# SebastianHafner/multimodal_siamese_cd

Measured on AMD Instinct MI355X. Metric: image-pairs/sec training step, 256×256 SAR+optical Siamese U-Net, 1/2/4/8 MI355X, higher is better.
Workload: dtype f32 (h2 split-fp16); 1 GPU; baseline_siamese: siameseunet TOPOLOGY [64, 128, 256, 512], 5-ch SAR+optical, 256x256, bs=32/GPU, conv math h2, fp32 activation storage, train step incl. AdamW; global_batch=32, tile=256, parallelism=dp1

## Files before the change

### include/scd.h

```cpp
#ifndef SCD_H_
#define SCD_H_

#include <stddef.h>
#include <stdint.h>

#ifdef __cplusplus
extern "C" {
#endif

typedef void *scd_stream_t;

enum scd_status {
    SCD_OK = 0,
    SCD_ERR_ARG = -1,
    SCD_ERR_ALIGN = -2,
    SCD_ERR_LAUNCH = -3,
    SCD_ERR_DEVICE = -4,
    SCD_ERR_WORKSPACE = -5,
};

enum scd_dtype {
    SCD_DT_F32 = 0,
    SCD_DT_BF16 = 1
};

typedef struct scd_nhwc {
    void *data;
    int32_t n, h, w, c, ldc;
    int32_t dtype;
} scd_nhwc_t;

const char *scd_version(void);
const char *scd_last_error(void);
int scd_device_check(int device);

int scd_pack_nchw(const float *src, int32_t n, int32_t c, int32_t h, int32_t w, int32_t c_begin,
                  int32_t c_count, scd_nhwc_t dst, float *bound, scd_stream_t stream);

typedef struct scd_pack_job {
    const float *w;
    float *out;
    uint16_t *split;
    int32_t co, ci, ci_pad, mode;
    int32_t math;
} scd_pack_job_t;
int scd_pack_conv3x3_multi(const scd_pack_job_t *jobs, int32_t n, scd_stream_t stream);
int scd_pack_conv3x3(const float *w, int32_t co, int32_t ci, int32_t ci_pad, int32_t mode, float *out,
                     scd_stream_t stream);

int scd_pack_convT2x2(const float *w, int32_t ci, int32_t co, int32_t mode, float *out, scd_stream_t stream);
int scd_pack_convT2x2_multi(const scd_pack_job_t *jobs, int32_t n, scd_stream_t stream);

enum scd_conv_math {
    SCD_MATH_F32 = 0,
    SCD_MATH_X3 = 1,
    SCD_MATH_BF16 = 2,
    SCD_MATH_X5 = 3,
    SCD_MATH_H2 = 4
};
#define SCD_ABI_VERSION 11
int scd_abi_version(void);
#define SCD_TUNE_HALO16_CFG(id)   ((uint32_t)((id) + 1))
#define SCD_TUNE_HALO16_OFF       0xFu
#define SCD_TUNE_HALO16_MASK      0xFu
#define SCD_TUNE_HALO16_WRING     0x8u
#define SCD_TUNE_H2_TILE_2X2      (1u << 4)
#define SCD_TUNE_H2_TILE64_2X2    (1u << 5)
#define SCD_TUNE_H2_NO_PRESCALE   (1u << 6)
#define SCD_TUNE_NO_XCD_REMAP     (1u << 7)
#define SCD_TUNE_HALO_ORDER_M     (1u << 8)
#define SCD_TUNE_W16_LAYOUT_2X2   (1u << 9)
#define SCD_TUNE_WGRAD_R64        (1u << 10)
#define SCD_TUNE_BF16_1XN         (1u << 11)
#define SCD_TUNE_X3_TILE(t)       ((uint32_t)(t) << 12)
#define SCD_TUNE_X3_TILE_MASK     (0xFu << 12)
#define SCD_TUNE_C16_TILES(k)     ((uint32_t)(k) << 16)
#define SCD_TUNE_C16_TILES_MASK   (0xFu << 16)
#define SCD_TUNE_HALO16_DB_OFF    (1u << 20)
#define SCD_TUNE_HALO16_DB_ON     (1u << 21)
#define SCD_TUNE_NO_GATHER16      (1u << 22)
#define SCD_TUNE_NO_WGRAD_C16     (1u << 23)
#define SCD_TUNE_NO_WGRAD_H2      (1u << 24)
#define SCD_TUNE_NO_HALO16_C16    (1u << 25)
#define SCD_TUNE_NO_HALO          (1u << 26)
#define SCD_TUNE_H2_TILE64_128    (1u << 28)
#define SCD_TUNE_WGRAD16_REGSTAGE (1u << 30)
int scd_split_bf16x3(const float *src, int64_t n, uint16_t *dst, scd_stream_t stream);
size_t scd_split_frag_bytes(int32_t n_out, int32_t K);
int scd_split_bf16x3_frag(const float *w, int32_t n_out, int32_t K, uint16_t *dst, scd_stream_t stream);
int scd_split_h2_frag(const float *w, int32_t n_out, int32_t K, uint16_t *dst, scd_stream_t stream);

typedef struct scd_bn_bwd_tiles {
    scd_nhwc_t y;
    int32_t nseg;
    const float *save_mean, *save_invstd, *scale, *shift;
    float *rec;
} scd_bn_bwd_tiles_t;

typedef struct scd_igemm {
    scd_nhwc_t src;
    int32_t out_h, out_w;
    int32_t stride;
    int32_t ntaps;
    int8_t dy[9], dx[9];
    const float *wpk;
    int32_t n_out;
    const float *bias;
    scd_nhwc_t dst;
    int32_t store_mode;
    const uint16_t *wsplit;
    float *stat_rec;
    const float *in_scale;
    const float *in_shift;
    int32_t in_nseg;
    const scd_bn_bwd_tiles_t *bn_bwd;
    const float *src_bound;
    float *dst_bound;
    int32_t math;
    uint32_t tune;
    const float *dst_bound_seed;
} scd_igemm_t;

int scd_conv_igemm(const scd_igemm_t *d, scd_stream_t stream);
int scd_igemm_arith(const scd_igemm_t *d);
int scd_igemm_bn_bwd_tiles(const scd_igemm_t *d, int32_t *tile_pixels);
int scd_igemm_input_bn_supported(const scd_igemm_t *d);
int scd_igemm_stat_tiles(const scd_igemm_t *d, int32_t *tile_pixels);

enum scd_igemm_family {
    SCD_KERNEL_F32 = 0,
    SCD_KERNEL_X3 = 1,
    SCD_KERNEL_HALO32 = 2,
    SCD_KERNEL_HALO16 = 3,
    SCD_KERNEL_HALO16_C16 = 4,
    SCD_KERNEL_GATHER16 = 5
};
typedef struct scd_igemm_kernel {
    int32_t family;
    int32_t layout;
    int32_t block_pixels;
    int32_t block_channels;
    int32_t tile_width;
    int32_t np;
    int32_t db;
    int32_t sb;
    int32_t in_bn;
    int32_t wl;
} scd_igemm_kernel_t;
int scd_igemm_kernel(const scd_igemm_t *d, scd_igemm_kernel_t *out);

typedef struct scd_wgrad {
    scd_nhwc_t rows;
    scd_nhwc_t src;
    int32_t stride;
    int32_t ntaps;
    int8_t dy[9], dx[9];
    const float *src_scale;
    const float *src_shift;
    int32_t src_nseg;
    const float *rows_bound;
    const float *src_bound;
    scd_nhwc_t rows_y;
    int32_t rows_nseg;
    const float *rows_mean, *rows_invstd, *rows_gamma, *rows_scale, *rows_shift, *rows_coef;
    int32_t math;
    uint32_t tune;
    float *src_colsum;
// ... 253 lines not shown
```

### multimodal_siamese_cd_amd/csrc/conv_halo16.hip

```cpp
#include "x3_common.h"

namespace scd {

template <int CTRL>
__device__ __forceinline__ float dpp_mov(float x) {
    return __builtin_bit_cast(float, __builtin_amdgcn_update_dpp(0, __builtin_bit_cast(int, x), CTRL, 0xf, 0xf, false));
}
__device__ __forceinline__ float row16_sum(float x) {
    x += dpp_mov<0x140>(x);
    x += dpp_mov<0x141>(x);
    x += dpp_mov<0xB1>(x);
    x += dpp_mov<0x4E>(x);
    return x;
}

__device__ __forceinline__ f32x4 row16_sum4(f32x4 v) {
    float a, b, c, d;
    asm volatile(
        "s_nop 1\n\t"
        "v_add_f32_dpp %0, %4, %4 row_mirror row_mask:0xf bank_mask:0xf bound_ctrl:1\n\t"
        "v_add_f32_dpp %1, %5, %5 row_mirror row_mask:0xf bank_mask:0xf bound_ctrl:1\n\t"
        "v_add_f32_dpp %2, %6, %6 row_mirror row_mask:0xf bank_mask:0xf bound_ctrl:1\n\t"
        "v_add_f32_dpp %3, %7, %7 row_mirror row_mask:0xf bank_mask:0xf bound_ctrl:1\n\t"
        "v_add_f32_dpp %0, %0, %0 row_half_mirror row_mask:0xf bank_mask:0xf bound_ctrl:1\n\t"
// ... 1040 lines not shown
}

template <int TW>
static void launch_c16_tw(const IgemmArgs &b, dim3 grid, hipStream_t s) {
    switch (c16_planes(b)) {
        case 1:
            if (b.sb)
                hipLaunchKernelGGL((igemm_halo16_c16<TW, 1, true>), grid, dim3(256), 0, s, b);
            else
                hipLaunchKernelGGL((igemm_halo16_c16<TW, 1>), grid, dim3(256), 0, s, b);
            break;
        case 4: hipLaunchKernelGGL((igemm_halo16_c16<TW, 4>), grid, dim3(256), 0, s, b); break;
        case 5: hipLaunchKernelGGL((igemm_halo16_c16<TW, 5>), grid, dim3(256), 0, s, b); break;
        default: hipLaunchKernelGGL((igemm_halo16_c16<TW, 3>), grid, dim3(256), 0, s, b);
    }
}

template <int TW>
static int c16_resident(const IgemmArgs &b) {
    static int cache[4] = {0, 0, 0, 0};
    const int pl = c16_planes(b);
    const int k = pl == 1 ? 0 : pl == 5 ? 1 : pl == 4 ? 3 : 2;
    if (cache[k] > 0) return cache[k];
    const void *fn = k == 0   ? reinterpret_cast<const void *>(&igemm_halo16_c16<TW, 1>)
                     : k == 1 ? reinterpret_cast<const void *>(&igemm_halo16_c16<TW, 5>)
                     : k == 3 ? reinterpret_cast<const void *>(&igemm_halo16_c16<TW, 4>)
                              : reinterpret_cast<const void *>(&igemm_halo16_c16<TW, 3>);
    int per_cu = 0, cus = 0, dev = 0;
    if (hipGetDevice(&dev) != hipSuccess ||
        hipDeviceGetAttribute(&cus, hipDeviceAttributeMultiprocessorCount, dev) != hipSuccess ||
        hipOccupancyMaxActiveBlocksPerMultiprocessor(&per_cu, fn, 256, 0) != hipSuccess || per_cu < 1 || cus < 1) {
        (void)hipGetLastError();
        cache[k] = 2 * 256;
        return cache[k];
    }
    cache[k] = per_cu * cus;
    return cache[k];
}

void launch_halo16_c16(const IgemmArgs &a, int tw, hipStream_t s) {
    IgemmArgs b = a;
    b.grid_m = a.n_img * (a.ho / (128 / tw)) * (a.wo / tw);
    b.grid_n = (a.n_out + 63) / 64;
    b.remap = 0;
    const int64_t ntile = int64_t(b.grid_m) * b.grid_n;
    const int cap = tw == 64 ? c16_resident<64>(a) : tw == 32 ? c16_resident<32>(a) : c16_resident<16>(a);
    const int kt = int((a.tune & SCD_TUNE_C16_TILES_MASK) >> 16);
    const int k = kt == 0 ? 4 : kt == 15 ? 0 : kt;
    const int64_t blocks = k >= 1 ? (ntile + k - 1) / k : (ntile < cap ? ntile : cap);
    const dim3 grid(static_cast<unsigned>(blocks));
    if (tw == 64)
        launch_c16_tw<64>(b, grid, s);
    else if (tw == 32)
        launch_c16_tw<32>(b, grid, s);
    else
        launch_c16_tw<16>(b, grid, s);
}

namespace {
constexpr int kW16RS = 160;

#ifndef SCD_WGRAD_ROW_WALK
#define SCD_WGRAD_ROW_WALK 0
#endif
__device__ __forceinline__ int patch_y0(int pr, int pw_n, int ph_n, int ph) {
    return SCD_WGRAD_ROW_WALK ? (pr / pw_n) * ph : (pr - (pr / ph_n) * ph_n) * ph;
}
__device__ __forceinline__ int patch_x0(int pr, int pw_n, int ph_n, int pw) {
    return SCD_WGRAD_ROW_WALK ? (pr - (pr / pw_n) * pw_n) * pw : (pr / ph_n) * pw;
}

template <int NP>
constexpr int w16_xp() { return NP == 1 ? 1 : (NP == 5 || NP == 2 || NP == 4) ? 2 : 3; }
template <int NP>
constexpr int w16_dp() { return NP == 1 ? 1 : (NP == 2 || NP == 4) ? 2 : 3; }

template <int LC>
struct W16L {
    static constexpr int CB = LC ? 1 : 2;
    static constexpr int RB = LC ? 4 : 2;
    static constexpr int NH = 9 * CB;
};

template <int T, int CB, int PB, int HW_, int NP>
__device__ __forceinline__ void w16_read_x(s16x4 (&f)[6], uint32_t xbase) {
    constexpr int toff = (T / 3) * HW_ + (T % 3);
    tr_read<0 * PB + toff * kW16RS + CB * 32>(f[0], xbase);
    tr_read<0 * PB + (toff + 8) * kW16RS + CB * 32>(f[1], xbase);
    if constexpr (w16_xp<NP>() >= 2) {
        tr_read<1 * PB + toff * kW16RS + CB * 32>(f[2], xbase);
        tr_read<1 * PB + (toff + 8) * kW16RS + CB * 32>(f[3], xbase);
    }
    if constexpr (w16_xp<NP>() == 3) {
        tr_read<2 * PB + toff * kW16RS + CB * 32>(f[4], xbase);
        tr_read<2 * PB + (toff + 8) * kW16RS + CB * 32>(f[5], xbase);
    }
}

template <int I, int PA, int NRB, int DP, int RSD>
__device__ __forceinline__ void w16_read_dy(bf16x8 (&dv)[3][NRB], uint32_t dbase) {
    if constexpr (I < DP * NRB) {
        constexpr int p = I / NRB, rb = I % NRB;
        s16x4 lo, hi;
        tr_read<p * PA + rb * 32>(lo, dbase);
        tr_read<p * PA + 8 * RSD + rb * 32>(hi, dbase);
        dv[p][rb] = cat8(lo, hi);
        w16_read_dy<I + 1, PA, NRB, DP, RSD>(dv, dbase);
    }
}

template <int T, int CB, int WAIT, int NP, int LC>
__device__ __forceinline__ void w16_half(f32x4 (&acc)[9][W16L<LC>::CB][W16L<LC>::RB],
                                         bf16x8 (&dv)[3][W16L<LC>::RB], s16x4 (&f)[6]) {
    bf16x8 x0 = cat8(f[0], f[1]), x1 = cat8(f[2], f[3]), x2 = cat8(f[4], f[5]);
    if constexpr (NP == 2 || NP == 4) {
        lds_wait<WAIT>(x0, x1);
        if (T == 0 && CB == 0) {
#pragma unroll
            for (int rb = 0; rb < W16L<LC>::RB; ++rb) lds_wait<WAIT>(dv[0][rb], dv[1][rb]);
        }
        const u32x4 xh = __builtin_bit_cast(u32x4, x0), xm = __builtin_bit_cast(u32x4, x1);
        const u32x4 xh_lo = NP == 4 ? f16_down11(xh) : xh;
#pragma unroll
        for (int rb = 0; rb < W16L<LC>::RB; ++rb) {
            const u32x4 dh = __builtin_bit_cast(u32x4, dv[0][rb]), dm = __builtin_bit_cast(u32x4, dv[1][rb]);
            acc[T][CB][rb] = mfma16_f16(xm, dh, acc[T][CB][rb]);
            acc[T][CB][rb] = mfma16_f16(xh_lo, dm, acc[T][CB][rb]);
            acc[T][CB][rb] = mfma16_f16(xh, dh, acc[T][CB][rb]);
        }
        return;
    }
    if constexpr (NP != 1) {
        if constexpr (NP == 3)
            lds_wait<WAIT>(x0, x1, x2);
        else
            lds_wait<WAIT>(x0, x1);
        if (T == 0 && CB == 0) {
#pragma unroll
            for (int rb = 0; rb < W16L<LC>::RB; ++rb) lds_wait<WAIT>(dv[0][rb], dv[1][rb], dv[2][rb]);
        }
    } else {
        lds_wait<WAIT>(x0);
        if (T == 0 && CB == 0) {
#pragma unroll
            for (int rb = 0; rb < W16L<LC>::RB; ++rb) lds_wait<WAIT>(dv[0][rb]);
        }
    }
#pragma unroll
    for (int rb = 0; rb < W16L<LC>::RB; ++rb) {
        if constexpr (NP != 1) {
            acc[T][CB][rb] = __builtin_amdgcn_mfma_f32_16x16x32_bf16(x1, dv[1][rb], acc[T][CB][rb], 0, 0, 0);
            acc[T][CB][rb] = __builtin_amdgcn_mfma_f32_16x16x32_bf16(x0, dv[2][rb], acc[T][CB][rb], 0, 0, 0);
            if constexpr (NP == 3)
                acc[T][CB][rb] = __builtin_amdgcn_mfma_f32_16x16x32_bf16(x2, dv[0][rb], acc[T][CB][rb], 0, 0, 0);
            acc[T][CB][rb] = __builtin_amdgcn_mfma_f32_16x16x32_bf16(x0, dv[1][rb], acc[T][CB][rb], 0, 0, 0);
            acc[T][CB][rb] = __builtin_amdgcn_mfma_f32_16x16x32_bf16(x1, dv[0][rb], acc[T][CB][rb], 0, 0, 0);
        }
        acc[T][CB][rb] = __builtin_amdgcn_mfma_f32_16x16x32_bf16(x0, dv[0][rb], acc[T][CB][rb], 0, 0, 0);
    }
}

template <int H, int PB, int HW_, int NP, int LC>
__device__ __forceinline__ void w16_chain(f32x4 (&acc)[9][W16L<LC>::CB][W16L<LC>::RB], bf16x8 (&dv)[3][W16L<LC>::RB],
                                          s16x4 (&f0)[6], s16x4 (&f1)[6], uint32_t xbase) {
    constexpr int NCB = W16L<LC>::CB, NH = W16L<LC>::NH;
    if constexpr (H < NH) {
        s16x4 (&f)[6] = (H & 1) ? f1 : f0;
        w16_half<H / NCB, H % NCB, (H == NH - 1 ? 0 : 2 * w16_xp<NP>()), NP, LC>(acc, dv, f);
        if constexpr (H + 2 < NH) w16_read_x<(H + 2) / NCB, (H + 2) % NCB, PB, HW_, NP>(f, xbase);
        w16_chain<H + 1, PB, HW_, NP, LC>(acc, dv, f0, f1, xbase);
    }
}

constexpr int kW16PH = 2, kW16PW = 16;

struct W16Block {
    int split, ct, r0, c0;
    int pw_n, ph_n, pimg, pbeg, pend;
    bool writer;
};
template <int ROWS, int COLS, bool RBN>
__device__ __forceinline__ W16Block w16_block(const WgradArgs &a) {
    W16Block b;
    const uint32_t per_split = COLS == 16 ? uint32_t(a.grid_r) : uint32_t(a.grid_r * a.grid_j);
    const uint32_t L = a.remap ? xcd_swizzle(blockIdx.x, gridDim.x) : blockIdx.x;
    b.split = int(L / per_split);
    const int rem = int(L - uint32_t(b.split) * per_split);
    b.ct = COLS == 16 ? 0 : rem / a.grid_r;
    b.r0 = (rem - b.ct * a.grid_r) * ROWS;
    b.c0 = b.ct * COLS;
    b.pw_n = a.wo / kW16PW;
    b.ph_n = a.ho / kW16PH;
    b.pimg = b.pw_n * b.ph_n;
    const int npatch = a.n_img_w * b.pimg;
    b.pbeg = b.split * a.kchunk;
    b.pend = min(npatch, b.pbeg + a.kchunk);
    b.writer = RBN && a.rows_out && b.ct == 0;
    return b;
}

template <int NCB, int NRB>
__device__ __forceinline__ void w16_store_slabs(f32x4 (&acc)[9][NCB][NRB], const WgradArgs &a, int split, int r0w, int w16,
                                                int c0w, int g) {
    float *slab = a.slabs + size_t(split) * a.R * a.Ng;
#pragma unroll
    for (int t = 0; t < 9; ++t)
#pragma unroll
        for (int cb = 0; cb < NCB; ++cb)
#pragma unroll
            for (int r = 0; r < NRB; ++r) {
                const int row = r0w + 16 * r + w16;
                const int col = c0w + 16 * cb + 4 * g;
                gstore4(slab + size_t(row) * a.Ng + t * a.C + col, acc[t][cb][r]);
            }
}
}

template <int NP, int LC, int RG, bool SB = false, bool RBN = false>
__global__ __launch_bounds__(256 * RG, 2 / RG) void wgrad_halo16_x3(WgradArgs a) {
    static_assert(!SB || NP == 1, "bf16 storage runs the bf16 arithmetic");
    static_assert(!RBN || (LC == 1 && (NP == 1 || NP == 4)), "rows transform: h2 / bf16, along-c layout");
    constexpr uint32_t EB = SB ? 2u : 4u;
    constexpr int NT = 256 * RG;
    constexpr int PH = kW16PH, PW = kW16PW, P = PH * PW;
    constexpr int HW_ = PW + 2, HP = (PH + 2) * HW_;
    constexpr int RS = kW16RS;
    constexpr int RSD = 128 * RG + 32;
    constexpr int CQ = 16 * RG;
    constexpr int PA = P * RSD, PB = HP * RS;
    constexpr int A_CH = P * CQ, B_CH = HP * 16;
    constexpr int A_PER = A_CH / NT, B_PER = (B_CH + NT - 1) / NT;
    static_assert(RG == 1 || (RG == 2 && LC == 1), "128-row blocks use the along-c wave layout");
    static_assert(NP == 1 || NP == 2 || NP == 3 || NP == 4 || NP == 5, "x3, x5, bf16 or h2");
    constexpr bool H2 = NP == 2 || NP == 4;
    constexpr int DP = w16_dp<NP>();
    constexpr int XP = w16_xp<NP>();
    constexpr int STAGE = DP * PA + XP * PB;
    constexpr int RBLK = 64 * RG;
    constexpr int COEF = RBN ? 2 * 7 * RBLK * 4 : 0;
    constexpr bool YDMA = RBN && H2;
    constexpr int YST = YDMA ? A_PER * NT * 16 : 0;
    __shared__ __attribute__((aligned(16))) unsigned char smem[STAGE + COEF + YST];
    float ds = 1.f, ds_inv = 1.f, xs = 1.f, xs_inv = 1.f;
    if constexpr (H2) {
        h2_scale(*a.rows_bound, ds, ds_inv);
        h2_scale(*a.src_bound, xs, xs_inv);
    }

    const int tid = threadIdx.x, lane = tid & 63, wid = tid >> 6;
    constexpr int NCB = W16L<LC>::CB, NRB = W16L<LC>::RB;
    const int wi = LC ? (RG == 1 ? 0 : wid >> 2) : wid >> 1, wj = LC ? (RG == 1 ? wid : wid & 3) : wid & 1;
    const W16Block blk = w16_block<RBLK, 64, RBN>(a);
    const int r0 = blk.r0, c0 = blk.c0, pimg = blk.pimg, pbeg = blk.pbeg, pend = blk.pend;

    const __amdgpu_buffer_rsrc_t rs_rows = make_rsrc(a.rows, a.rows_bytes);
    const __amdgpu_buffer_rsrc_t rs_src = make_rsrc(a.src, a.src_bytes);
    const __amdgpu_buffer_rsrc_t rs_y = make_rsrc(RBN ? a.rows_y : a.rows, RBN ? a.y_bytes : 0u);
    const bool writer = blk.writer;
    float omax = 0.f;

    StageT<SB> ra[A_PER], rb[B_PER], ya[RBN && !YDMA ? A_PER : 1];
    unsigned char *const ystage = smem + STAGE + COEF;
    const int wave_u = __builtin_amdgcn_readfirstlane(wid);
    f32x4 x_sc, x_sh;
    uint32_t x_valid = 0;
    int st_img = 0, st_y0 = 0, st_x0 = 0;
    auto load_patch = [&](int pi) {
        const int img = pi / pimg, pr = pi - img * pimg;
        if (a.src_scale) {
            const int ch = (img / a.src_seg_imgs) * a.C + c0 + (tid & 15) * 4;
            x_sc = gload4(a.src_scale + ch);
            x_sh = gload4(a.src_shift + ch);
        }
        x_valid = 0;
        const int y0 = patch_y0(pr, blk.pw_n, blk.ph_n, PH), x0 = patch_x0(pr, blk.pw_n, blk.ph_n, PW);
        st_img = img;
        st_y0 = y0;
        st_x0 = x0;
#pragma unroll
        for (int i = 0; i < A_PER; ++i) {
            const int e = tid + i * NT, q = e / CQ, cq = e % CQ;
            const int py = q >> 4, px = q & 15;
            const int pix = (img * a.ho + y0 + py) * a.wo + x0 + px;
            if constexpr (YDMA)
                __builtin_amdgcn_global_load_lds(
                    (const __attribute__((address_space(1))) void *)(a.rows_y + size_t(pix) * a.ldc_y + r0 + cq * 4),
                    (__attribute__((address_space(3))) void *)(ystage + (i * NT + wave_u * 64) * 16), 16, 0, 0);
            ra[i] = bload_q<SB>(rs_rows, uint32_t(pix * a.ldc_r + r0 + cq * 4) * EB);
            if constexpr (RBN && !YDMA) ya[i] = bload_q<SB>(rs_y, uint32_t(pix * a.ldc_y + r0 + cq * 4) * EB);
        }
#pragma unroll
        for (int i = 0; i < B_PER; ++i) {
            const int e = tid + i * NT, hp = e >> 4, cq = e & 15;
            const int hy = hp / HW_, hx = hp - (hp / HW_) * HW_;
            const int sy = y0 - 1 + hy, sx = x0 - 1 + hx;
            const bool v = e < B_CH && unsigned(sy) < unsigned(a.hs) && unsigned(sx) < unsigned(a.ws);
            x_valid |= uint32_t(v) << i;
            rb[i] = bload_q<SB>(rs_src, v ? uint32_t(((img * a.hs + sy) * a.ws + sx) * a.ldc_s + c0 + cq * 4) * EB : kOOB);
        }
    };
    auto store_patch = [&]() {
        const f32x4 sc = H2 ? x_sc * xs : x_sc, sh = H2 ? x_sh * xs : x_sh;
        if constexpr (YDMA) asm volatile("s_waitcnt vmcnt(0)" ::: "memory");
#pragma unroll
        for (int i = 0; i < A_PER; ++i) {
            const int e = tid + i * NT;
            const int o = (e / CQ) * RSD + (e % CQ) * 8;
            u32x2 h, m, l;
            if constexpr (RBN) {
                const int cq = e % CQ, q = e / CQ;
                const float *cf =
                    reinterpret_cast<const float *>(smem + STAGE) + (st_img / a.rows_seg_imgs) * 7 * RBLK + cq * 4;
                const f32x4 mu = *reinterpret_cast<const f32x4 *>(cf), iv = *reinterpret_cast<const f32x4 *>(cf + RBLK);
                const f32x4 sc = *reinterpret_cast<const f32x4 *>(cf + 2 * RBLK);
                const f32x4 sf = *reinterpret_cast<const f32x4 *>(cf + 3 * RBLK);
                const f32x4 k1 = *reinterpret_cast<const f32x4 *>(cf + 4 * RBLK);
                const f32x4 k2 = *reinterpret_cast<const f32x4 *>(cf + 5 * RBLK);
                const f32x4 mul = *reinterpret_cast<const f32x4 *>(cf + 6 * RBLK);
                f32x4 yv;
                if constexpr (YDMA)
                    yv = *reinterpret_cast<const f32x4 *>(ystage + e * 16);
                else
                    yv = stage_f32<SB>(ya[i]);
                f32x4 dv = bn_bwd_dy4(yv, stage_f32<SB>(ra[i]), mu, iv, sc, sf, k1, k2, mul);
                if constexpr (SB) {
                    const u32x2 bits = pk_bf16x4(dv);
                    ra[i] = bits;
                    dv = unpk_bf16x4(bits);
                } else {
                    ra[i] = dv;
                }
                if (writer) {
                    const int pix = (st_img * a.ho + st_y0 + (q >> 4)) * a.wo + st_x0 + (q & 15);
                    const size_t idx = size_t(pix) * a.ldc_o + r0 + cq * 4;
                    if constexpr (SB)
                        *reinterpret_cast<u32x2 *>(static_cast<unsigned short *>(a.rows_out) + idx) = ra[i];
                    else
                        gstore4(static_cast<float *>(a.rows_out) + idx, dv);
                    omax = fmaxf(omax, fmaxf(fmaxf(fabsf(dv[0]), fabsf(dv[1])), fmaxf(fabsf(dv[2]), fabsf(dv[3]))));
                }
            }
            if constexpr (H2) {
                if constexpr (NP == 4)
                    split2h_pre(ra[i] * ds, h, m);
                else
                    split2h(ra[i] * ds, h, m);
                *reinterpret_cast<u32x2 *>(smem + PA + o) = m;
            } else if constexpr (DP == 3) {
                split3(ra[i], h, m, l);
                *reinterpret_cast<u32x2 *>(smem + PA + o) = m;
                *reinterpret_cast<u32x2 *>(smem + 2 * PA + o) = l;
            } else {
                h = stage_bits<SB>(ra[i]);
            }
            *reinterpret_cast<u32x2 *>(smem + o) = h;
        }
#pragma unroll
        for (int i = 0; i < B_PER; ++i)
            if constexpr (SB) {
                if (tid + i * NT < B_CH) {
                    u32x2 h = rb[i];
                    if (a.src_scale) {
                        const bool v = (x_valid >> i) & 1u;
                        f32x4 x = unpk_bf16x4(rb[i]);
#pragma unroll
                        for (int q = 0; q < 4; ++q) x[q] = v ? fmaxf(fmaf(x[q], sc[q], sh[q]), 0.f) : 0.f;
                        h = pk_bf16x4(x);
                    }
                    const int e = tid + i * NT;
                    *reinterpret_cast<u32x2 *>(smem + DP * PA + (e >> 4) * RS + (e & 15) * 8) = h;
                }
            } else if (tid + i * NT < B_CH) {
                u32x2 h, m, l;
                if (a.src_scale) {
                    const bool v = (x_valid >> i) & 1u;
#pragma unroll
                    for (int q = 0; q < 4; ++q) rb[i][q] = v ? fmaxf(fmaf(rb[i][q], sc[q], sh[q]), 0.f) : 0.f;
                } else if constexpr (H2) {
                    rb[i] *= xs;
                }
                const int e = tid + i * NT;
                const int o = DP * PA + (e >> 4) * RS + (e & 15) * 8;
                if constexpr (H2) {
                    split2h(rb[i], h, m);
                    *reinterpret_cast<u32x2 *>(smem + PB + o) = m;
                } else if constexpr (XP >= 2) {
                    split3(rb[i], h, m, l);
                    *reinterpret_cast<u32x2 *>(smem + PB + o) = m;
                    if constexpr (XP == 3) *reinterpret_cast<u32x2 *>(smem + 2 * PB + o) = l;
                } else {
                    h[0] = cvt_pk_bf16(rb[i][0], rb[i][1]);
                    h[1] = cvt_pk_bf16(rb[i][2], rb[i][3]);
                }
                *reinterpret_cast<u32x2 *>(smem + o) = h;
            }
    };

    f32x4 acc[9][NCB][NRB];
#pragma unroll
    for (int t = 0; t < 9; ++t)
#pragma unroll
        for (int i = 0; i < NCB; ++i)
#pragma unroll
            for (int j = 0; j < NRB; ++j) acc[t][i][j] = f32x4{0.f, 0.f, 0.f, 0.f};

    const int g = lane >> 4, w16 = lane & 15;
    const int py = g >> 1, pxq = 4 * (g & 1) + (w16 >> 2);
    const uint32_t dbase = lds_addr(smem) + (py * PW + pxq) * RSD + (16 * NRB * wi + 4 * (w16 & 3)) * 2;
    const uint32_t xbase = lds_addr(smem) + DP * PA + (py * HW_ + pxq) * RS + (16 * NCB * wj + 4 * (w16 & 3)) * 2;

    if constexpr (RBN) {
        float *cf = reinterpret_cast<float *>(smem + STAGE);
        const int nsl = a.n_img_w / a.rows_seg_imgs;
        for (int e = tid; e < nsl * RBLK; e += NT) {
            const int sg = e / RBLK, r = e - sg * RBLK, o = sg * a.R + r0 + r;
            const float iv = a.rbn_inv[o];
            float *c = cf + sg * 7 * RBLK + r;
            c[0] = a.rbn_mean[o];
            c[RBLK] = iv;
            c[2 * RBLK] = a.rbn_scale[o];
            c[3 * RBLK] = a.rbn_shift[o];
            c[4 * RBLK] = a.rbn_coef[2 * o];
            c[5 * RBLK] = a.rbn_coef[2 * o + 1];
            c[6 * RBLK] = (a.rbn_gamma ? a.rbn_gamma[r0 + r] : 1.f) * iv;
        }
        __syncthreads();
    }
    if (pbeg < pend) {
        load_patch(pbeg);
        store_patch();
        __syncthreads();
        for (int pi = pbeg; pi < pend; ++pi) {
            const bool more = pi + 1 < pend;
            if (more) load_patch(pi + 1);
            bf16x8 dv[3][NRB];
            w16_read_dy<0, PA, NRB, DP, RSD>(dv, dbase);
            s16x4 f0[6], f1[6];
            w16_read_x<0 / NCB, 0 % NCB, PB, HW_, NP>(f0, xbase);
            w16_read_x<1 / NCB, 1 % NCB, PB, HW_, NP>(f1, xbase);
            w16_chain<0, PB, HW_, NP, LC>(acc, dv, f0, f1, xbase);
            if (more) {
                __syncthreads();
                store_patch();
                __syncthreads();
            }
        }
    }

    if constexpr (H2) {
        const float k = ds_inv * xs_inv;
#pragma unroll
        for (int t = 0; t < 9; ++t)
#pragma unroll
            for (int cb = 0; cb < NCB; ++cb)
#pragma unroll
                for (int r = 0; r < NRB; ++r) acc[t][cb][r] *= k;
    }
    if (writer && a.rows_out_bound) wave_max_bound(a.rows_out_bound, omax);
    w16_store_slabs(acc, a, blk.split, r0 + 16 * NRB * wi, w16, c0 + 16 * NCB * wj, g);
}

namespace {
constexpr int kDmaSink = 1024;
}
#ifndef SCD_WGRAD16_DMA_NB
#define SCD_WGRAD16_DMA_NB 4
#endif
#ifndef SCD_WGRAD16_DMA_TRANSFORMS
#define SCD_WGRAD16_DMA_TRANSFORMS 1
#endif
#ifndef SCD_WGRAD16_DMA_NB_XT
#define SCD_WGRAD16_DMA_NB_XT 5
#endif

template <int RG, int NB, bool XT = false, bool RBN = false>
__global__ __launch_bounds__(256 * RG, 2 / RG) void wgrad_halo16_dma(WgradArgs a) {
    constexpr int NT = 256 * RG, NW = NT / 64;
    constexpr int PH = kW16PH, PW = kW16PW, P = PH * PW;
    constexpr int HW_ = PW + 2, HP = (PH + 2) * HW_;
    constexpr int RS = kW16RS;
    constexpr int RSD = 128 * RG + 32;
    constexpr int PA = P * RSD, PB = HP * RS;
    constexpr int PA_K = (PA + 1023) / 1024, PB_K = (PB + 1023) / 1024;
    constexpr int NPC = PA_K + PB_K + (RBN ? PA_K : 0);
    constexpr int PPW = (NPC + NW - 1) / NW;
    constexpr int STAGE = NPC * 1024;
    constexpr int DCH = 8 * RG;
    constexpr int RBLK = 64 * RG;
    constexpr int NCB = W16L<1>::CB, NRB = W16L<1>::RB;
    constexpr bool TR = XT || RBN;
    static_assert(NB >= (TR ? 3 : 2) && NB <= 6, "ring depth");
    static_assert(!RBN || (P * DCH) % NT == 0, "rows transform: whole 16-byte chunks per thread");
    constexpr int RCH = RBN ? P * DCH / NT : 0;
    constexpr int CFX = XT ? 2 * 2 * 64 * 4 : 0;
    constexpr int CFR = RBN ? 2 * 7 * RBLK * 4 : 0;
    static_assert(NB * STAGE + kDmaSink + CFX + CFR <= 160 * 1024,
                  "ring depth NB: NB patch buffers and the coefficient tables exceed the CU's 160 KB of LDS");
    __shared__ __attribute__((aligned(16))) unsigned char smem[NB * STAGE + kDmaSink + CFX + CFR];

    const int tid = threadIdx.x, lane = tid & 63, wid = tid >> 6;
    const int wave_u = __builtin_amdgcn_readfirstlane(wid);
    const int wi = RG == 1 ? 0 : wid >> 2, wj = RG == 1 ? wid : wid & 3;
    const W16Block blk = w16_block<RBLK, 64, RBN>(a);
    const int r0 = blk.r0, c0 = blk.c0, pimg = blk.pimg, pbeg = blk.pbeg, pend = blk.pend;
    const bool writer = blk.writer;
    float omax = 0.f;

    const __amdgpu_buffer_rsrc_t rs_rows = make_rsrc(a.rows, a.rows_bytes);
    const __amdgpu_buffer_rsrc_t rs_src = make_rsrc(a.src, a.src_bytes);
    const __amdgpu_buffer_rsrc_t rs_y = make_rsrc(RBN ? a.rows_y : a.rows, RBN ? a.y_bytes : 0u);
    int rel[PPW], x_hy[PPW], x_hx[PPW], kind[PPW];
#pragma unroll
    for (int k = 0; k < PPW; ++k) {
        const int u = k * NW + wave_u;
        kind[k] = 2;
        rel[k] = x_hy[k] = x_hx[k] = 0;
        const bool is_y = RBN && u >= PA_K + PB_K && u < NPC;
        if (u < PA_K || is_y) {
            const int b = (is_y ? u - PA_K - PB_K : u) * 1024 + lane * 16;
            const int row = b / RSD, ch = (b - row * RSD) / 16;
            if (row < P && ch < DCH) {
                kind[k] = 0;
                rel[k] = ((row >> 4) * a.wo + (row & 15)) * (is_y ? a.ldc_y : a.ldc_r) + r0 + 8 * ch;
            }
        } else if (u < PA_K + PB_K) {
            const int b = (u - PA_K) * 1024 + lane * 16;
// ... 148 lines not shown
            cfx[sg * 128 + c] = a.src_scale[sg * a.C + c0 + c];
            cfx[sg * 128 + 64 + c] = a.src_shift[sg * a.C + c0 + c];
        }
    }
    if constexpr (RBN) {
        const int nsl = a.n_img_w / a.rows_seg_imgs;
        for (int e = tid; e < nsl * RBLK; e += NT) {
            const int sg = e / RBLK, r = e - sg * RBLK, o = sg * a.R + r0 + r;
            const float iv = a.rbn_inv[o];
            float *c = cfr + sg * 7 * RBLK + r;
            c[0] = a.rbn_mean[o];
            c[RBLK] = iv;
            c[2 * RBLK] = a.rbn_scale[o];
            c[3 * RBLK] = a.rbn_shift[o];
            c[4 * RBLK] = a.rbn_coef[2 * o];
            c[5 * RBLK] = a.rbn_coef[2 * o + 1];
            c[6 * RBLK] = (a.rbn_gamma ? a.rbn_gamma[r0 + r] : 1.f) * iv;
        }
    }

    const int wst = writer ? RCH : 0;
    Cursor ci = cursor_at(pbeg), ct1 = ci;
#pragma unroll
    for (int k = 0; k < NB - 1; ++k)
        if (pbeg + k < pend) {
            issue(ci, k);
            advance(ci);
        }
    if constexpr (TR) {
        if (pbeg < pend) {
            const int ahead = min(NB - 2, pend - 1 - pbeg);
            if (ahead >= 3)
                asm volatile("s_waitcnt vmcnt(%0)" ::"n"(3 * PPW) : "memory");
            else if (ahead == 2)
                asm volatile("s_waitcnt vmcnt(%0)" ::"n"(2 * PPW) : "memory");
            else if (ahead == 1)
                asm volatile("s_waitcnt vmcnt(%0)" ::"n"(PPW) : "memory");
            else
                asm volatile("s_waitcnt vmcnt(0)" ::: "memory");
            lds_barrier();
            transform(ct1, 0);
            advance(ct1);
        }
    }
    int slot = 0;
    for (int pi = pbeg; pi < pend; ++pi) {
        const int ahead = TR ? (pi + 1 < pend ? min(NB - 3, pend - 2 - pi) : -1) : min(NB - 2, pend - 1 - pi);
        if (wst == 0) {
            if (ahead >= 4)
                asm volatile("s_waitcnt vmcnt(%0)" ::"n"(4 * PPW) : "memory");
            else if (ahead == 3)
                asm volatile("s_waitcnt vmcnt(%0)" ::"n"(3 * PPW) : "memory");
            else if (ahead == 2)
                asm volatile("s_waitcnt vmcnt(%0)" ::"n"(2 * PPW) : "memory");
            else if (ahead == 1)
                asm volatile("s_waitcnt vmcnt(%0)" ::"n"(PPW) : "memory");
            else if (ahead == 0)
                asm volatile("s_waitcnt vmcnt(0)" ::: "memory");
        } else if constexpr (RBN) {
            if (ahead >= 3)
                asm volatile("s_waitcnt vmcnt(%0)" ::"n"(3 * PPW + RCH) : "memory");
            else if (ahead == 2)
                asm volatile("s_waitcnt vmcnt(%0)" ::"n"(2 * PPW + RCH) : "memory");
            else if (ahead == 1)
                asm volatile("s_waitcnt vmcnt(%0)" ::"n"(PPW + RCH) : "memory");
            else if (ahead == 0)
                asm volatile("s_waitcnt vmcnt(%0)" ::"n"(RCH) : "memory");
        }
        lds_barrier();
        if (pi + NB - 1 < pend) {
            issue(ci, slot == 0 ? NB - 1 : slot - 1);
            advance(ci);
        }
        if constexpr (TR) {
            if (pi + 1 < pend) {
                transform(ct1, slot == NB - 1 ? 0 : slot + 1);
                advance(ct1);
            }
        }
        const uint32_t bo = uint32_t(slot * STAGE);
        bf16x8 dv[3][NRB];
        w16_read_dy<0, PA_K * 1024, NRB, 1, RSD>(dv, dbase + bo);
        s16x4 f0[6], f1[6];
        w16_read_x<0, 0, PB_K * 1024, HW_, 1>(f0, xbase + bo);
        w16_read_x<1, 0, PB_K * 1024, HW_, 1>(f1, xbase + bo);
        w16_chain<0, PB_K * 1024, HW_, 1, 1>(acc, dv, f0, f1, xbase + bo);
        slot = slot == NB - 1 ? 0 : slot + 1;
    }
    asm volatile("s_waitcnt vmcnt(0)" ::: "memory");
    if (writer && a.rows_out_bound) wave_max_bound(a.rows_out_bound, omax);
    w16_store_slabs(acc, a, blk.split, r0 + 16 * NRB * wi, w16, c0 + 16 * NCB * wj, g);
}

namespace {
constexpr int kC16RS = 32;

template <int T, int PB, int HW_, int NP>
__device__ __forceinline__ void c16_read_x(s16x4 (&f)[6], uint32_t xbase) {
    constexpr int toff = (T / 3) * HW_ + (T % 3);
    tr_read<0 * PB + toff * kC16RS>(f[0], xbase);
    tr_read<0 * PB + (toff + 8) * kC16RS>(f[1], xbase);
    if constexpr (w16_xp<NP>() >= 2) {
        tr_read<1 * PB + toff * kC16RS>(f[2], xbase);
        tr_read<1 * PB + (toff + 8) * kC16RS>(f[3], xbase);
    }
    if constexpr (w16_xp<NP>() == 3) {
        tr_read<2 * PB + toff * kC16RS>(f[4], xbase);
        tr_read<2 * PB + (toff + 8) * kC16RS>(f[5], xbase);
    }
}

template <int T, int WAIT, int NP>
__device__ __forceinline__ void c16_tap(f32x4 (&acc)[9], bf16x8 (&dv)[3], s16x4 (&f)[6]) {
    bf16x8 x0 = cat8(f[0], f[1]), x1 = cat8(f[2], f[3]), x2 = cat8(f[4], f[5]);
    if constexpr (NP == 4) {
        lds_wait<WAIT>(x0, x1);
        if (T == 0) lds_wait<WAIT>(dv[0], dv[1]);
        const u32x4 xh = __builtin_bit_cast(u32x4, x0), xm = __builtin_bit_cast(u32x4, x1);
        const u32x4 dh = __builtin_bit_cast(u32x4, dv[0]), dm = __builtin_bit_cast(u32x4, dv[1]);
        acc[T] = mfma16_f16(xm, dh, acc[T]);
        acc[T] = mfma16_f16(f16_down11(xh), dm, acc[T]);
        acc[T] = mfma16_f16(xh, dh, acc[T]);
        return;
    }
    if constexpr (NP != 1) {
        if constexpr (NP == 3)
            lds_wait<WAIT>(x0, x1, x2);
        else
            lds_wait<WAIT>(x0, x1);
        if (T == 0) lds_wait<WAIT>(dv[0], dv[1], dv[2]);
    } else {
        lds_wait<WAIT>(x0, dv[0]);
    }
    if constexpr (NP != 1) {
        acc[T] = __builtin_amdgcn_mfma_f32_16x16x32_bf16(x1, dv[1], acc[T], 0, 0, 0);
        acc[T] = __builtin_amdgcn_mfma_f32_16x16x32_bf16(x0, dv[2], acc[T], 0, 0, 0);
        if constexpr (NP == 3) acc[T] = __builtin_amdgcn_mfma_f32_16x16x32_bf16(x2, dv[0], acc[T], 0, 0, 0);
        acc[T] = __builtin_amdgcn_mfma_f32_16x16x32_bf16(x0, dv[1], acc[T], 0, 0, 0);
        acc[T] = __builtin_amdgcn_mfma_f32_16x16x32_bf16(x1, dv[0], acc[T], 0, 0, 0);
    }
    acc[T] = __builtin_amdgcn_mfma_f32_16x16x32_bf16(x0, dv[0], acc[T], 0, 0, 0);
}

template <int T, int PB, int HW_, int NP>
__device__ __forceinline__ void c16_chain(f32x4 (&acc)[9], bf16x8 (&dv)[3], s16x4 (&f0)[6], s16x4 (&f1)[6],
                                          uint32_t xbase) {
    if constexpr (T < 9) {
        s16x4 (&f)[6] = (T & 1) ? f1 : f0;
        c16_tap<T, (T == 8 ? 0 : 2 * w16_xp<NP>()), NP>(acc, dv, f);
        if constexpr (T + 2 < 9) c16_read_x<T + 2, PB, HW_, NP>(f, xbase);
        c16_chain<T + 1, PB, HW_, NP>(acc, dv, f0, f1, xbase);
    }
}
}

template <int NP, bool RBN, bool SB = false>
__global__ __launch_bounds__(256, 2) void wgrad_halo16_c16(WgradArgs a) {
    static_assert(!SB || NP == 1, "bf16 storage runs the bf16 arithmetic");
    constexpr uint32_t EB = SB ? 2u : 4u;
    constexpr int PH = kW16PH, PW = kW16PW, P = PH * PW;
    constexpr int HW_ = PW + 2, HP = (PH + 2) * HW_;
    constexpr int RS = kW16RS, RSX = kC16RS;
    constexpr int PA = P * RS, PB = HP * RSX;
    constexpr int A_CH = P * 16, B_CH = HP * 4;
    constexpr int A_PER = A_CH / 256, B_PER = (B_CH + 255) / 256;
    static_assert(NP == 1 || NP == 3 || NP == 4 || NP == 5, "x3, x5, bf16 or h2");
    constexpr bool H2 = NP == 4;
    constexpr int DP = w16_dp<NP>();
    constexpr int XP = w16_xp<NP>();
// ... 339 lines not shown
```

### multimodal_siamese_cd_amd/hip.py

```python
from __future__ import annotations

import collections
import contextlib
import contextvars
import ctypes
import os
from ctypes import POINTER, c_char_p, c_float, c_int, c_int8, c_int32, c_int64, c_size_t, c_uint8, c_uint32, c_void_p

import torch

LIB_PATH = os.environ.get("SCD_LIB") or os.path.join(os.path.dirname(os.path.abspath(__file__)), "_lib", "libscd.so")


class NHWC(ctypes.Structure):

    _fields_ = [("data", c_void_p), ("n", c_int32), ("h", c_int32), ("w", c_int32), ("c", c_int32), ("ldc", c_int32),
                ("dtype", c_int32)]


DT_F32, DT_BF16 = 0, 1
_VIEW_DTYPES = {torch.float32: (DT_F32, 4), torch.bfloat16: (DT_BF16, 2)}


class BNBWD(ctypes.Structure):
# ... 365 lines not shown
    out = torch.empty(ci * co * 4, device=w.device, dtype=torch.float32)
    _check(lib().scd_pack_convT2x2(w.contiguous().data_ptr(), ci, co, mode, out.data_ptr(), _stream()),
           "scd_pack_convT2x2")
    return _attach_split(out, 4 * co, ci, 1) if mode == 0 else _attach_split(out, ci, 4 * co, 4)


def pack_convT2x2_multi(jobs) -> list:
    if not jobs:
        return []
    split = conv_math() != 'f32'
    m = _MATH_NAMES[conv_math()]
    outs, keep, arr = [], [], (PACKJOB * len(jobs))()
    for i, (w, mode) in enumerate(jobs):
        ci, co = w.shape[0], w.shape[1]
        w = w.contiguous()
        n_out, K = (4 * co, ci) if mode == 0 else (ci, 4 * co)
        out = torch.empty(ci * co * 4, device=w.device, dtype=torch.float32)
        sp = None
        if split and K % 16 == 0:
            sp = torch.empty(lib().scd_split_frag_bytes(n_out, K) // 2, dtype=torch.int16, device=w.device)
            out._x3 = sp
        keep.append(w)
        arr[i] = PACKJOB(w.data_ptr(), out.data_ptr(), _ptr(sp), co, ci, ci, mode, m)
        outs.append(out)
    _check(lib().scd_pack_convT2x2_multi(ctypes.cast(arr, c_void_p), len(jobs), _stream()), "scd_pack_convT2x2_multi")
    return outs


def split_bf16x3(src: torch.Tensor) -> torch.Tensor:
    n = src.numel()
    dst = torch.empty(3 * n, dtype=torch.int16, device=src.device)
    _check(lib().scd_split_bf16x3(src.data_ptr(), n, dst.data_ptr(), _stream()), "scd_split_bf16x3")
    return dst


def split_h2_frag(wpk: torch.Tensor, n_out: int, K: int) -> torch.Tensor:
    nbytes = lib().scd_split_frag_bytes(n_out, K)
    dst = torch.empty(nbytes // 2, dtype=torch.int16, device=wpk.device)
    _check(lib().scd_split_h2_frag(wpk.data_ptr(), n_out, K, dst.data_ptr(), _stream()), "scd_split_h2_frag")
    return dst


def split_bf16x3_frag(wpk: torch.Tensor, n_out: int, K: int) -> torch.Tensor:
    nbytes = lib().scd_split_frag_bytes(n_out, K)
    dst = torch.empty(nbytes // 2, dtype=torch.int16, device=wpk.device)
    _check(lib().scd_split_bf16x3_frag(wpk.data_ptr(), n_out, K, dst.data_ptr(), _stream()), "scd_split_bf16x3_frag")
    return dst


def h2_weight_format(K: int, ntaps: int) -> bool:
    if conv_math() != 'h2' or ntaps not in (9, 1, 4) or K % ntaps:
        return False
    c = K // ntaps
    return c % 32 == 0 or (ntaps == 9 and c == 16)


def _attach_split(wpk: torch.Tensor, n_out: int, K: int, ntaps: int) -> torch.Tensor:
    if K % 16 == 0 and conv_math() != 'f32':
        wpk._x3 = split_h2_frag(wpk, n_out, K) if h2_weight_format(K, ntaps) else split_bf16x3_frag(wpk, n_out, K)
    return wpk


MATH_F32, MATH_X3, MATH_BF16, MATH_X5, MATH_H2 = 0, 1, 2, 3, 4
_MATH_NAMES = {'f32': MATH_F32, 'x3': MATH_X3, 'bf16': MATH_BF16, 'x5': MATH_X5, 'h2': MATH_H2}
_MATH_BY_ID = {v: k for k, v in _MATH_NAMES.items()}

TUNE_HALO16_OFF = 0xF
TUNE_HALO16_WRING = 0x8
TUNE_H2_TILE_2X2 = 1 << 4
TUNE_H2_TILE64_2X2 = 1 << 5
TUNE_H2_NO_PRESCALE = 1 << 6
TUNE_NO_XCD_REMAP = 1 << 7
TUNE_HALO_ORDER_M = 1 << 8
TUNE_W16_LAYOUT_2X2 = 1 << 9
TUNE_WGRAD_R64 = 1 << 10
TUNE_BF16_1XN = 1 << 11
TUNE_HALO16_DB_OFF = 1 << 20
TUNE_HALO16_DB_ON = 1 << 21
TUNE_NO_GATHER16 = 1 << 22
TUNE_NO_WGRAD_C16 = 1 << 23
TUNE_NO_WGRAD_H2 = 1 << 24
TUNE_NO_HALO16_C16 = 1 << 25
TUNE_NO_HALO = 1 << 26
TUNE_H2_TILE64_128 = 1 << 28
TUNE_WGRAD16_REGSTAGE = 1 << 30


def tune_halo16_cfg(tile_id: int) -> int:
    return tile_id + 1


def tune_x3_tile(t: int) -> int:
    return (t & 15) << 12


def tune_c16_tiles(k: int) -> int:
    return (k & 15) << 16


_DEFAULT = {'math': MATH_X3, 'tune': 0}
_SCOPE: contextvars.ContextVar = contextvars.ContextVar('scd_conv_scope', default=None)


def _cur():
    sc = _SCOPE.get()
    return sc if sc is not None else (_DEFAULT['math'], _DEFAULT['tune'])


def _math_id(mode) -> int:
    if isinstance(mode, str):
        if mode not in _MATH_NAMES:
            raise ValueError(f"conv arithmetic {mode!r}: expected one of {sorted(_MATH_NAMES)}")
        return _MATH_NAMES[mode]
    m = int(mode)
    if m not in _MATH_BY_ID:
        raise ValueError(f"conv arithmetic {mode!r}")
    return m


def conv_math() -> str:
    return _MATH_BY_ID[_cur()[0]]


def conv_tune() -> int:
    return _cur()[1]


@contextlib.contextmanager
def conv_scope(math=None, tune=None):
    m0, t0 = _cur()
    tok = _SCOPE.set((m0 if math is None else _math_id(math), t0 if tune is None else int(tune)))
    try:
        yield
    finally:
        _SCOPE.reset(tok)


def set_conv_math(mode) -> str:
    prev = _MATH_BY_ID[_DEFAULT['math']]
    _DEFAULT['math'] = _math_id(mode)
    return prev


def set_tune(bits: int) -> int:
    prev = _DEFAULT['tune']
    _DEFAULT['tune'] = int(bits)
    return prev


def get_tune() -> int:
    return _DEFAULT['tune']


def set_halo16(mode: int) -> int:
    t = _DEFAULT['tune']
    v = t & 0xF
    prev = 0 if v == TUNE_HALO16_OFF else 1 if v in (0, TUNE_HALO16_WRING) else v + 1
    new = TUNE_HALO16_OFF if mode == 0 else 0 if mode == 1 else tune_halo16_cfg(int(mode) - 2)
    _DEFAULT['tune'] = (t & ~0xF) | new
    return prev


def halo16_tile_width_pref() -> int:
    return 16


# ... 583 lines not shown
```

Before: 1091 image-pairs/s.

## Reuse halo rows across vertically adjacent patches in wgrad16 via LDS row ring

In the 16-wide weight-gradient kernel (RG==1), consecutive patches walking down a column share two halo rows of the input. The input tile is kept as a ring of row pairs in LDS, so each new patch loads and stores only the two new rows instead of all four. The x-read helpers now take per-row base addresses so the 3x3 taps can index the rotated ring. This cuts global loads and LDS stores for the input, at the cost of extra address selection, phase bookkeeping, and a more complex first-patch path. It can be disabled with a new tune flag.

Result: no change. 1098 image-pairs/s (median of 6 runs) (+0.7%).

```diff
diff --git a/include/scd.h b/include/scd.h
--- a/include/scd.h
+++ b/include/scd.h
@@ -83,6 +83,7 @@
 #define SCD_TUNE_NO_WGRAD_H2      (1u << 24)
 #define SCD_TUNE_NO_HALO16_C16    (1u << 25)
 #define SCD_TUNE_NO_HALO          (1u << 26)
+#define SCD_TUNE_WGRAD16_NO_ROLL  (1u << 27)
 #define SCD_TUNE_H2_TILE64_128    (1u << 28)
 #define SCD_TUNE_WGRAD16_REGSTAGE (1u << 30)
 int scd_split_bf16x3(const float *src, int64_t n, uint16_t *dst, scd_stream_t stream);
diff --git a/multimodal_siamese_cd_amd/csrc/conv_halo16.hip b/multimodal_siamese_cd_amd/csrc/conv_halo16.hip
--- a/multimodal_siamese_cd_amd/csrc/conv_halo16.hip
+++ b/multimodal_siamese_cd_amd/csrc/conv_halo16.hip
@@ -1146,18 +1146,33 @@
     static constexpr int NH = 9 * CB;
 };
 
-template <int T, int CB, int PB, int HW_, int NP>
-__device__ __forceinline__ void w16_read_x(s16x4 (&f)[6], uint32_t xbase) {
-    constexpr int toff = (T / 3) * HW_ + (T % 3);
-    tr_read<0 * PB + toff * kW16RS + CB * 32>(f[0], xbase);
-    tr_read<0 * PB + (toff + 8) * kW16RS + CB * 32>(f[1], xbase);
+struct W16XRing {
+    uint32_t row[3];
+    static constexpr int kRowStep = 0;
+    template <int DY>
+    __device__ __forceinline__ uint32_t base() const { return row[DY]; }
+};
+template <int HW_>
+struct W16XLinear {
+    uint32_t b;
+    static constexpr int kRowStep = HW_ * kW16RS;
+    template <int DY>
+    __device__ __forceinline__ uint32_t base() const { return b; }
+};
+
+template <int T, int CB, int PB, int NP, class XB>
+__device__ __forceinline__ void w16_read_x(s16x4 (&f)[6], const XB &xb) {
+    constexpr int toff = (T / 3) * XB::kRowStep + (T % 3) * kW16RS;
+    const uint32_t xrow = xb.template base<T / 3>();
+    tr_read<0 * PB + toff + CB * 32>(f[0], xrow);
+    tr_read<0 * PB + toff + 8 * kW16RS + CB * 32>(f[1], xrow);
     if constexpr (w16_xp<NP>() >= 2) {
-        tr_read<1 * PB + toff * kW16RS + CB * 32>(f[2], xbase);
-        tr_read<1 * PB + (toff + 8) * kW16RS + CB * 32>(f[3], xbase);
+        tr_read<1 * PB + toff + CB * 32>(f[2], xrow);
+        tr_read<1 * PB + toff + 8 * kW16RS + CB * 32>(f[3], xrow);
     }
     if constexpr (w16_xp<NP>() == 3) {
-        tr_read<2 * PB + toff * kW16RS + CB * 32>(f[4], xbase);
-        tr_read<2 * PB + (toff + 8) * kW16RS + CB * 32>(f[5], xbase);
+        tr_read<2 * PB + toff + CB * 32>(f[4], xrow);
+        tr_read<2 * PB + toff + 8 * kW16RS + CB * 32>(f[5], xrow);
     }
 }
 
@@ -1224,15 +1239,15 @@
     }
 }
 
-template <int H, int PB, int HW_, int NP, int LC>
+template <int H, int PB, int NP, int LC, class XB>
 __device__ __forceinline__ void w16_chain(f32x4 (&acc)[9][W16L<LC>::CB][W16L<LC>::RB], bf16x8 (&dv)[3][W16L<LC>::RB],
-                                          s16x4 (&f0)[6], s16x4 (&f1)[6], uint32_t xbase) {
+                                          s16x4 (&f0)[6], s16x4 (&f1)[6], const XB &xb) {
     constexpr int NCB = W16L<LC>::CB, NH = W16L<LC>::NH;
     if constexpr (H < NH) {
         s16x4 (&f)[6] = (H & 1) ? f1 : f0;
         w16_half<H / NCB, H % NCB, (H == NH - 1 ? 0 : 2 * w16_xp<NP>()), NP, LC>(acc, dv, f);
-        if constexpr (H + 2 < NH) w16_read_x<(H + 2) / NCB, (H + 2) % NCB, PB, HW_, NP>(f, xbase);
-        w16_chain<H + 1, PB, HW_, NP, LC>(acc, dv, f0, f1, xbase);
+        if constexpr (H + 2 < NH) w16_read_x<(H + 2) / NCB, (H + 2) % NCB, PB, NP>(f, xb);
+        w16_chain<H + 1, PB, NP, LC>(acc, dv, f0, f1, xb);
     }
 }
 
@@ -1292,8 +1307,11 @@
     constexpr int RSD = 128 * RG + 32;
     constexpr int CQ = 16 * RG;
     constexpr int PA = P * RSD, PB = HP * RS;
-    constexpr int A_CH = P * CQ, B_CH = HP * 16;
-    constexpr int A_PER = A_CH / NT, B_PER = (B_CH + NT - 1) / NT;
+    constexpr int PAIR = 2 * HW_ * RS;
+    constexpr int A_CH = P * CQ, B_ROW = HW_ * 16;
+    constexpr int A_PER = A_CH / NT;
+    constexpr bool ROLLS = RG == 1;
+    constexpr int B_PER = ((ROLLS ? 2 : 4) * B_ROW + NT - 1) / NT;
     static_assert(RG == 1 || (RG == 2 && LC == 1), "128-row blocks use the along-c wave layout");
     static_assert(NP == 1 || NP == 2 || NP == 3 || NP == 4 || NP == 5, "x3, x5, bf16 or h2");
     constexpr bool H2 = NP == 2 || NP == 4;
@@ -1329,18 +1347,38 @@
     f32x4 x_sc, x_sh;
     uint32_t x_valid = 0;
     int st_img = 0, st_y0 = 0, st_x0 = 0;
-    auto load_patch = [&](int pi) {
+    bool st_roll = false;
+#if SCD_WGRAD_ROW_WALK
+    const bool no_roll = true;
+#else
+    const bool no_roll = (a.tune & SCD_TUNE_WGRAD16_NO_ROLL) != 0;
+#endif
+    int phase = 0;
+    auto load_x = [&](int row0, int nrows) {
+        x_valid = 0;
+#pragma unroll
+        for (int i = 0; i < B_PER; ++i) {
+            const int e = tid + i * NT, hp = e >> 4, cq = e & 15;
+            const int hy = hp / HW_, hx = hp - (hp / HW_) * HW_;
+            const int sy = st_y0 - 1 + row0 + hy, sx = st_x0 - 1 + hx;
+            const bool v = e < nrows * B_ROW && unsigned(sy) < unsigned(a.hs) && unsigned(sx) < unsigned(a.ws);
+            x_valid |= uint32_t(v) << i;
+            rb[i] =
+                bload_q<SB>(rs_src, v ? uint32_t(((st_img * a.hs + sy) * a.ws + sx) * a.ldc_s + c0 + cq * 4) * EB : kOOB);
+        }
+    };
+    auto load_patch = [&](int pi, bool first) {
         const int img = pi / pimg, pr = pi - img * pimg;
         if (a.src_scale) {
             const int ch = (img / a.src_seg_imgs) * a.C + c0 + (tid & 15) * 4;
             x_sc = gload4(a.src_scale + ch);
             x_sh = gload4(a.src_shift + ch);
         }
-        x_valid = 0;
         const int y0 = patch_y0(pr, blk.pw_n, blk.ph_n, PH), x0 = patch_x0(pr, blk.pw_n, blk.ph_n, PW);
         st_img = img;
         st_y0 = y0;
         st_x0 = x0;
+        st_roll = ROLLS && !first && !no_roll && y0 != 0;
 #pragma unroll
         for (int i = 0; i < A_PER; ++i) {
             const int e = tid + i * NT, q = e / CQ, cq = e % CQ;
@@ -1353,18 +1391,9 @@
             ra[i] = bload_q<SB>(rs_rows, uint32_t(pix * a.ldc_r + r0 + cq * 4) * EB);
             if constexpr (RBN && !YDMA) ya[i] = bload_q<SB>(rs_y, uint32_t(pix * a.ldc_y + r0 + cq * 4) * EB);
         }
-#pragma unroll
-        for (int i = 0; i < B_PER; ++i) {
-            const int e = tid + i * NT, hp = e >> 4, cq = e & 15;
-            const int hy = hp / HW_, hx = hp - (hp / HW_) * HW_;
-            const int sy = y0 - 1 + hy, sx = x0 - 1 + hx;
-            const bool v = e < B_CH && unsigned(sy) < unsigned(a.hs) && unsigned(sx) < unsigned(a.ws);
-            x_valid |= uint32_t(v) << i;
-            rb[i] = bload_q<SB>(rs_src, v ? uint32_t(((img * a.hs + sy) * a.ws + sx) * a.ldc_s + c0 + cq * 4) * EB : kOOB);
-        }
+        load_x(st_roll ? 2 : 0, ROLLS ? 2 : 4);
     };
-    auto store_patch = [&]() {
-        const f32x4 sc = H2 ? x_sc * xs : x_sc, sh = H2 ? x_sh * xs : x_sh;
+    auto store_dy = [&]() {
         if constexpr (YDMA) asm volatile("s_waitcnt vmcnt(0)" ::: "memory");
 #pragma unroll
         for (int i = 0; i < A_PER; ++i) {
@@ -1419,10 +1448,14 @@
             }
             *reinterpret_cast<u32x2 *>(smem + o) = h;
         }
+    };
+    auto store_x = [&](int ring0, int nrows) {
+        const f32x4 sc = H2 ? x_sc * xs : x_sc, sh = H2 ? x_sh * xs : x_sh;
+        unsigned char *const xp = smem + DP * PA + ring0 * (HW_ * RS);
 #pragma unroll
         for (int i = 0; i < B_PER; ++i)
             if constexpr (SB) {
-                if (tid + i * NT < B_CH) {
+                if (tid + i * NT < nrows * B_ROW) {
                     u32x2 h = rb[i];
                     if (a.src_scale) {
                         const bool v = (x_valid >> i) & 1u;
@@ -1432,9 +1465,9 @@
                         h = pk_bf16x4(x);
                     }
                     const int e = tid + i * NT;
-                    *reinterpret_cast<u32x2 *>(smem + DP * PA + (e >> 4) * RS + (e & 15) * 8) = h;
-                }
-            } else if (tid + i * NT < B_CH) {
+                    *reinterpret_cast<u32x2 *>(xp + (e >> 4) * RS + (e & 15) * 8) = h;
+                }
+            } else if (tid + i * NT < nrows * B_ROW) {
                 u32x2 h, m, l;
                 if (a.src_scale) {
                     const bool v = (x_valid >> i) & 1u;
@@ -1444,20 +1477,33 @@
                     rb[i] *= xs;
                 }
                 const int e = tid + i * NT;
-                const int o = DP * PA + (e >> 4) * RS + (e & 15) * 8;
+                const int o = (e >> 4) * RS + (e & 15) * 8;
                 if constexpr (H2) {
                     split2h(rb[i], h, m);
-                    *reinterpret_cast<u32x2 *>(smem + PB + o) = m;
+                    *reinterpret_cast<u32x2 *>(xp + PB + o) = m;
                 } else if constexpr (XP >= 2) {
                     split3(rb[i], h, m, l);
-                    *reinterpret_cast<u32x2 *>(smem + PB + o) = m;
-                    if constexpr (XP == 3) *reinterpret_cast<u32x2 *>(smem + 2 * PB + o) = l;
+                    *reinterpret_cast<u32x2 *>(xp + PB + o) = m;
+                    if constexpr (XP == 3) *reinterpret_cast<u32x2 *>(xp + 2 * PB + o) = l;
                 } else {
                     h[0] = cvt_pk_bf16(rb[i][0], rb[i][1]);
                     h[1] = cvt_pk_bf16(rb[i][2], rb[i][3]);
                 }
-                *reinterpret_cast<u32x2 *>(smem + o) = h;
-            }
+                *reinterpret_cast<u32x2 *>(xp + o) = h;
+            }
+    };
+    auto store_patch = [&]() {
+        store_dy();
+        phase = st_roll ? phase ^ 1 : 0;
+        if constexpr (ROLLS) {
+            if (!st_roll) {
+                store_x(0, 2);
+                load_x(2, 2);
+            }
+            store_x(2 * (phase ^ 1), 2);
+        } else {
+            store_x(0, 4);
+        }
     };
 
     f32x4 acc[9][NCB][NRB];
@@ -1472,6 +1518,15 @@
     const int py = g >> 1, pxq = 4 * (g & 1) + (w16 >> 2);
     const uint32_t dbase = lds_addr(smem) + (py * PW + pxq) * RSD + (16 * NRB * wi + 4 * (w16 & 3)) * 2;
     const uint32_t xbase = lds_addr(smem) + DP * PA + (py * HW_ + pxq) * RS + (16 * NCB * wj + 4 * (w16 & 3)) * 2;
+    using XBase = std::conditional_t<ROLLS, W16XRing, W16XLinear<HW_>>;
+    auto ring_bases = [&](int ph) {
+        if constexpr (ROLLS) {
+            const uint32_t lo = xbase + (ph ? PAIR : 0), hi = xbase + (ph ? 0 : PAIR);
+            return W16XRing{{lo, py ? hi - HW_ * RS : lo + HW_ * RS, hi}};
+        } else {
+            return W16XLinear<HW_>{xbase};
+        }
+    };
 
     if constexpr (RBN) {
         float *cf = reinterpret_cast<float *>(smem + STAGE);
@@ -1491,21 +1546,23 @@
         __syncthreads();
     }
     if (pbeg < pend) {
-        load_patch(pbeg);
+        load_patch(pbeg, true);
         store_patch();
+        XBase xb = ring_bases(phase);
         __syncthreads();
         for (int pi = pbeg; pi < pend; ++pi) {
             const bool more = pi + 1 < pend;
-            if (more) load_patch(pi + 1);
+            if (more) load_patch(pi + 1, false);
             bf16x8 dv[3][NRB];
             w16_read_dy<0, PA, NRB, DP, RSD>(dv, dbase);
             s16x4 f0[6], f1[6];
-            w16_read_x<0 / NCB, 0 % NCB, PB, HW_, NP>(f0, xbase);
-            w16_read_x<1 / NCB, 1 % NCB, PB, HW_, NP>(f1, xbase);
-            w16_chain<0, PB, HW_, NP, LC>(acc, dv, f0, f1, xbase);
+            w16_read_x<0 / NCB, 0 % NCB, PB, NP>(f0, xb);
+            w16_read_x<1 / NCB, 1 % NCB, PB, NP>(f1, xb);
+            w16_chain<0, PB, NP, LC>(acc, dv, f0, f1, xb);
             if (more) {
                 __syncthreads();
                 store_patch();
+                xb = ring_bases(phase);
                 __syncthreads();
             }
         }
@@ -1820,9 +1877,10 @@
         bf16x8 dv[3][NRB];
         w16_read_dy<0, PA_K * 1024, NRB, 1, RSD>(dv, dbase + bo);
         s16x4 f0[6], f1[6];
-        w16_read_x<0, 0, PB_K * 1024, HW_, 1>(f0, xbase + bo);
-        w16_read_x<1, 0, PB_K * 1024, HW_, 1>(f1, xbase + bo);
-        w16_chain<0, PB_K * 1024, HW_, 1, 1>(acc, dv, f0, f1, xbase + bo);
+        const W16XLinear<HW_> xb{xbase + bo};
+        w16_read_x<0, 0, PB_K * 1024, 1>(f0, xb);
+        w16_read_x<1, 0, PB_K * 1024, 1>(f1, xb);
+        w16_chain<0, PB_K * 1024, 1, 1>(acc, dv, f0, f1, xb);
         slot = slot == NB - 1 ? 0 : slot + 1;
     }
     asm volatile("s_waitcnt vmcnt(0)" ::: "memory");
diff --git a/multimodal_siamese_cd_amd/hip.py b/multimodal_siamese_cd_amd/hip.py
--- a/multimodal_siamese_cd_amd/hip.py
+++ b/multimodal_siamese_cd_amd/hip.py
@@ -471,6 +471,7 @@
 TUNE_NO_WGRAD_H2 = 1 << 24
 TUNE_NO_HALO16_C16 = 1 << 25
 TUNE_NO_HALO = 1 << 26
+TUNE_WGRAD16_NO_ROLL = 1 << 27
 TUNE_H2_TILE64_128 = 1 << 28
 TUNE_WGRAD16_REGSTAGE = 1 << 30
 
```
